# nubot-nudt/MDGAT-matcher

Hardware: AMD Instinct MI355X
Metric: keypoint-pairs/sec (higher is better)
Workload: dtype f32 (products as 3 split-f16 MFMAs, fp32 accumulate)

## Files before the change

mdgat_matcher_amd/csrc/attention_stream.hip:

```cpp
#include "common.hpp"
#include <utility>

namespace {

typedef float f32x2 __attribute__((ext_vector_type(2)));
typedef f16x8 __attribute__((may_alias)) f16x8_a;
typedef f32x4 __attribute__((may_alias)) f32x4_a;

constexpr int BLK_BYTES = 4096 + 128;
constexpr int CHUNK_BYTES = 4 * BLK_BYTES;
constexpr int NSLOT = 4;
constexpr int OROW = 36;

struct StreamArgs {
    const _Float16* q16;
    const _Float16* k16;
    const _Float16* vt16;
    float* msg;
    int N, M, Npad, PP, cross, QT;
};

template <typename F, int... U>
__device__ __forceinline__ void for_each_unit(F&& f, std::integer_sequence<int, U...>) { (f(U), ...); }
template <int N, typename F>
__device__ __forceinline__ void for_units(F&& f) { for_each_unit(f, std::make_integer_sequence<int, N>{}); }

#define SLOT_END() __builtin_amdgcn_sched_barrier(0)

template <bool FAST, bool QK_ONLY = false>
__global__ __launch_bounds__(256, 2) void attention_stream_kernel(StreamArgs a) {
    extern __shared__ __attribute__((aligned(16))) char smem[];
    const int tid = threadIdx.x, lane = tid & 63;
    const int wave = __builtin_amdgcn_readfirstlane(tid >> 6);
    const int l31 = lane & 31, hi = lane >> 5;
    const int i0 = blockIdx.x;
    const int grp = (i0 / (8 * a.QT)) * 8 + (i0 & 7), qt = (i0 >> 3) % a.QT;
    const int head = grp & 3, side = (grp >> 2) & 1, b = grp >> 3;
    const int P = a.N + a.M;
    const int nq = side ? a.M : a.N, q_off = side ? a.N : 0;
    const int src = a.cross ? 1 - side : side;
    const int nk = src ? a.M : a.N, k_off = src ? a.N : 0;
    const int q0 = qt * 128;
    if (q0 >= nq) return;
    const int NCH = nk >> 6;
    const unsigned lds0 = (unsigned)(size_t)(__attribute__((address_space(3))) char*)smem;

    const int rl8 = lane >> 3, swz = (lane & 7) ^ rl8;
    const char* dbase;
    unsigned voff, pstride, cstride;
    if (wave < 2) {
        dbase = reinterpret_cast<const char*>(a.k16 + (((size_t)b * P + k_off + wave * 32) * 4 + head) * 64);
        voff = rl8 * 512 + swz * 16; pstride = 8 * 512; cstride = 64 * 512;
    } else {
        dbase = reinterpret_cast<const char*>(a.vt16 + (((size_t)b * 4 + head) * 2 + (wave - 2)) * 32 * a.PP + (src ? a.Npad : 0));
        voff = rl8 * a.PP * 2 + swz * 16; pstride = 8 * a.PP * 2; cstride = 128;
    }
    auto dma_chunk = [&](int ch) __attribute__((always_inline)) {
        if (FAST && wave == 3) return;
        if (QK_ONLY && wave >= 2) return;
        const char* s0 = dbase + (size_t)ch * cstride;
        const unsigned d0 = lds0 + (unsigned)(ch & (NSLOT - 1)) * CHUNK_BYTES + (unsigned)wave * BLK_BYTES;
#pragma unroll
        for (int p = 0; p < 4; ++p)
            asm volatile("s_mov_b32 m0, %0\n\ts_nop 0\n\tglobal_load_lds_dwordx4 %1, %2"
                         :: "s"(d0 + p * 1024 + ((p >> 1) & 1) * 128), "v"(voff), "s"(s0 + (size_t)p * pstride) : "memory");
    };

    const int krow = (l31 & ~12) | ((l31 & 4) << 1) | ((l31 & 8) >> 1);
    unsigned kofs[4], vofs[4];
#pragma unroll
    for (int i = 0; i < 4; ++i) {
        const int c = 2 * i + hi;
        kofs[i] = (krow >> 3) * 1024 + ((krow >> 4) & 1) * 128 + ((krow & 7) * 8 + (c ^ (krow & 7))) * 16;
        vofs[i] = (l31 >> 3) * 1024 + ((l31 >> 4) & 1) * 128 + ((l31 & 7) * 8 + (c ^ (l31 & 7))) * 16;
    }
    f16x8 kf[4];
    f16x8 vh[2], vl[2];
    auto kread = [&](int ch, int jb) __attribute__((always_inline)) {
        const char* base = smem + (ch & (NSLOT - 1)) * CHUNK_BYTES + jb * BLK_BYTES;
#pragma unroll
        for (int i = 0; i < (FAST ? 2 : 4); ++i) kf[i] = *reinterpret_cast<const f16x8_a*>(base + kofs[i]);
    };
    auto vread = [&](int ch, int i) __attribute__((always_inline)) {
        if (QK_ONLY) return;
        const char* base = smem + (ch & (NSLOT - 1)) * CHUNK_BYTES + 2 * BLK_BYTES;
        vh[i & 1] = *reinterpret_cast<const f16x8_a*>(base + vofs[i]);
        if (!FAST) vl[i & 1] = *reinterpret_cast<const f16x8_a*>(base + BLK_BYTES + vofs[i]);
    };

    const int qw = q0 + wave * 32;
    f16x8 qh[2], ql[2];
    {
        const int qrow = min(qw + l31, nq - 1);
        const _Float16* p = a.q16 + (((size_t)b * P + q_off + qrow) * 4 + head) * 64 + 8 * hi;
        qh[0] = *reinterpret_cast<const f16x8*>(p);
        qh[1] = *reinterpret_cast<const f16x8*>(p + 16);
        ql[0] = *reinterpret_cast<const f16x8*>(p + 32);
        ql[1] = *reinterpret_cast<const f16x8*>(p + 48);
    }
    dma_chunk(0);
    if (NCH > 1) dma_chunk(1);
    if (NCH > 2) dma_chunk(2);
    if (NCH > 2) asm volatile("s_waitcnt vmcnt(8)" ::: "memory");
    else if (NCH > 1) asm volatile("s_waitcnt vmcnt(4)" ::: "memory");
    else asm volatile("s_waitcnt vmcnt(0)" ::: "memory");
    __syncthreads();

    const float NEG_INF = -__builtin_inff();
    const f32x16 zero16 = {0.f, 0.f, 0.f, 0.f, 0.f, 0.f, 0.f, 0.f, 0.f, 0.f, 0.f, 0.f, 0.f, 0.f, 0.f, 0.f};
    f32x16 Sc[2];
    f32x16 A, X;
    f32x16 Om = zero16;
    f32x2 l2 = {0.f, 0.f};
    float mxa = NEG_INF, mxb = NEG_INF;

    auto qk = [&](int k) __attribute__((always_inline)) {
        if (k == 0) A = __builtin_amdgcn_mfma_f32_32x32x16_f16(kf[0], qh[0], zero16, 0, 0, 0);
        else if (FAST) { if (k == 2) A = __builtin_amdgcn_mfma_f32_32x32x16_f16(kf[1], qh[1], A, 0, 0, 0); }
        else if (k == 1) X = __builtin_amdgcn_mfma_f32_32x32x16_f16(kf[0], ql[0], zero16, 0, 0, 0);
        else if (k == 2) A = __builtin_amdgcn_mfma_f32_32x32x16_f16(kf[1], qh[1], A, 0, 0, 0);
        else if (k == 3) X = __builtin_amdgcn_mfma_f32_32x32x16_f16(kf[1], ql[1], X, 0, 0, 0);
        else if (k == 4) X = __builtin_amdgcn_mfma_f32_32x32x16_f16(kf[2], qh[0], X, 0, 0, 0);
        else X = __builtin_amdgcn_mfma_f32_32x32x16_f16(kf[3], qh[1], X, 0, 0, 0);
    };
    auto comb = [&](int jb, int u) __attribute__((always_inline)) {
        if (u < 2) {
#pragma unroll
            for (int r = 8 * u; r < 8 * u + 8; r += 2) {
                if (FAST) { Sc[jb][r] = A[r]; Sc[jb][r + 1] = A[r + 1]; continue; }
                const f32x2 v = f32x2{X[r], X[r + 1]} + f32x2{A[r], A[r + 1]};
                Sc[jb][r] = v[0]; Sc[jb][r + 1] = v[1];
            }
        } else {
            const int r0 = 8 * (u - 2);
            mxa = fmaxf(mxa, fmaxf(Sc[jb][r0], Sc[jb][r0 + 1]));
            mxb = fmaxf(mxb, fmaxf(Sc[jb][r0 + 2], Sc[jb][r0 + 3]));
            mxa = fmaxf(mxa, fmaxf(Sc[jb][r0 + 4], Sc[jb][r0 + 5]));
            mxb = fmaxf(mxb, fmaxf(Sc[jb][r0 + 6], Sc[jb][r0 + 7]));
        }
    };

    for_units<2>([&](int jb) __attribute__((always_inline)) {
        kread(0, jb);
        for_units<6>([&](int k) __attribute__((always_inline)) { qk(k); });
        for_units<4>([&](int u) __attribute__((always_inline)) { comb(jb, u); });
    });
    float m_run;
    {
        float mc = fmaxf(mxa, mxb);
        m_run = fmaxf(mc, __shfl_xor(mc, 32, 64));
    }

    float pv[8];
    f16x8 php[2], plp[2];
#pragma unroll
    for (int j = 0; j < 8; ++j) { php[1][j] = (_Float16)0.f; plp[1][j] = (_Float16)0.f; vh[1][j] = (_Float16)0.f; vl[1][j] = (_Float16)0.f; }
    float m11 = 0.f;
    typedef unsigned u32x4 __attribute__((ext_vector_type(4)));
    auto vs = [&](int i, int u) __attribute__((always_inline)) {
        if (QK_ONLY) return;
        const int jb = i >> 1, r0 = 8 * (i & 1), pb = i & 1;
        if (u == 0) {
#pragma unroll
            for (int j = 0; j < 8; j += 2) {
                const f32x2 d = f32x2{Sc[jb][r0 + j], Sc[jb][r0 + j + 1]} - f32x2{m11, m11};
                pv[j] = d[0]; pv[j + 1] = d[1];
            }
        } else if (u == 1 || u == 2) {
#pragma unroll
            for (int j = 4 * (u - 1); j < 4 * u; ++j) pv[j] = __builtin_amdgcn_exp2f(pv[j]);
        } else if (u == 3) {
#pragma unroll
            for (int j = 0; j < 8; j += 2) l2 += f32x2{pv[j], pv[j + 1]};
        } else if (u == 4) {
#pragma unroll
            for (int j = 0; j < 8; ++j) php[pb][j] = (_Float16)pv[j];
        } else if (FAST) {
        } else if (u == 5 || u == 6) {
            const u32x4 hp = __builtin_bit_cast(u32x4, php[pb]);
#pragma unroll
            for (int j = 2 * (u - 5); j < 2 * (u - 4); ++j) {
                asm("v_fma_mix_f32 %0, %1, 1.0, -%2 op_sel:[0,0,0] op_sel_hi:[0,0,1]" : "=v"(pv[2 * j]) : "v"(pv[2 * j]), "v"(hp[j]));
                asm("v_fma_mix_f32 %0, %1, 1.0, -%2 op_sel:[0,0,1] op_sel_hi:[0,0,1]" : "=v"(pv[2 * j + 1]) : "v"(pv[2 * j + 1]), "v"(hp[j]));
            }
        } else {
#pragma unroll
            for (int j = 0; j < 8; ++j) plp[pb][j] = (_Float16)pv[j];
        }
    };
    auto pvm = [&](int i, int k) __attribute__((always_inline)) {
        if (QK_ONLY) return;
        const int pb = i & 1;
        if (k == 0) Om = __builtin_amdgcn_mfma_f32_32x32x16_f16(vh[pb], php[pb], Om, 0, 0, 0);
        else if (FAST) {}
        else if (k == 1) Om = __builtin_amdgcn_mfma_f32_32x32x16_f16(vl[pb], php[pb], Om, 0, 0, 0);
        else Om = __builtin_amdgcn_mfma_f32_32x32x16_f16(vh[pb], plp[pb], Om, 0, 0, 0);
    };

    auto max_halves = [&](float v) __attribute__((always_inline)) {
        float a_ = v, b_ = v;
        asm volatile("s_nop 1\n\tv_permlane32_swap_b32 %0, %1\n\ts_nop 1" : "+v"(a_), "+v"(b_));
        return fmaxf(a_, b_);
    };
    float sc = 1.0f;
    auto chunk_body = [&](int c, auto next_tag) __attribute__((always_inline)) {
        constexpr bool NEXT = decltype(next_tag)::value;
        if (c + 2 < NCH) asm volatile("s_waitcnt vmcnt(4)" ::: "memory");
        else asm volatile("s_waitcnt vmcnt(0)" ::: "memory");
        __syncthreads();
        if (c + 3 < NCH) dma_chunk(c + 3);
        if (NEXT) kread(c + 1, 0);
        m11 = m_run - 11.0f;
        mxa = NEG_INF; mxb = NEG_INF;
        l2 *= sc;
        SLOT_END();
        pvm(3, 0); vs(0, 0); SLOT_END();
        pvm(3, 1); vs(0, 1); SLOT_END();
        pvm(3, 2); vread(c, 0); SLOT_END();
        for_units<6>([&](int k) __attribute__((always_inline)) {
            if (NEXT) qk(k);
            vs(0, 2 + k);
            if (k == 3) vread(c, 1);
            SLOT_END();
        });
        if (!__all(sc == 1.0f)) {
#pragma unroll
            for (int r = 0; r < 16; ++r) Om[r] *= sc;
        }
        SLOT_END();
        if (NEXT) kread(c + 1, 1);
        for_units<8>([&](int u) __attribute__((always_inline)) {
            if (u < 3) pvm(0, u);
            vs(1, u);
            if (NEXT && u >= 3 && u < 7) comb(0, u - 3);
            if (u == 5) vread(c, 2);
            SLOT_END();
        });
        for_units<8>([&](int u) __attribute__((always_inline)) {
            if (NEXT && u < 6) qk(u);
            SLOT_END();
            if (u >= 1 && u < 4) pvm(1, u - 1);
            vs(2, u);
            if (u == 6) vread(c, 3);
            SLOT_END();
        });
        for_units<8>([&](int u) __attribute__((always_inline)) {
            if (u < 3) pvm(2, u);
            vs(3, u);
            if (NEXT && u >= 3 && u < 7) comb(1, u - 3);
            SLOT_END();
        });
        if (NEXT) {
            float mc = fmaxf(mxa, mxb);
            mc = max_halves(mc);
            const float m_new = mc > m_run + 4.0f ? mc : m_run;
            sc = __builtin_amdgcn_exp2f(m_run - m_new);
            m_run = m_new;
        }
    };
    for (int c = 0; c + 1 < NCH; ++c) chunk_body(c, std::true_type{});
    chunk_body(NCH - 1, std::false_type{});
    for_units<3>([&](int k) __attribute__((always_inline)) { pvm(3, k); });
    if (QK_ONLY) {
        if (hi == 0 && qw + l31 < nq) a.msg[((size_t)b * P + q_off + qw + l31) * 128 + head * 32] = m_run;
        return;
    }

    float l = l2[0] + l2[1];
    l += __shfl_xor(l, 32, 64);
    const float inv_l = 1.0f / l;
    float* T = reinterpret_cast<float*>(smem + ((NCH + 2 - (wave >> 1)) & (NSLOT - 1)) * CHUNK_BYTES) + (wave & 1) * 32 * OROW;
#pragma unroll
    for (int g4 = 0; g4 < 4; ++g4) {
        f32x4 o;
#pragma unroll
        for (int j = 0; j < 4; ++j) o[j] = Om[4 * g4 + j] * inv_l;
        *reinterpret_cast<f32x4_a*>(T + l31 * OROW + 8 * g4 + 4 * hi) = o;
    }
    float* out = a.msg + ((size_t)b * P + q_off) * 128 + head * 32;
#pragma unroll
    for (int it = 0; it < 4; ++it) {
        const int row = it * 8 + (lane >> 3), cc = lane & 7;
        const f32x4 v = *reinterpret_cast<const f32x4_a*>(T + row * OROW + cc * 4);
        const int q = qw + row;
        if (q < nq) *reinterpret_cast<f32x4*>(out + (size_t)q * 128 + cc * 4) = v;
    }
}


template <int NQ>
__global__ __launch_bounds__(256, 2) void qk_phase_probe_kernel(StreamArgs a) {
    extern __shared__ __attribute__((aligned(16))) char smem[];
    const int tid = threadIdx.x, lane = tid & 63;
    const int wave = __builtin_amdgcn_readfirstlane(tid >> 6);
    const int l31 = lane & 31, hi = lane >> 5;
    const int i0 = blockIdx.x;
    const int grp = (i0 / (8 * a.QT)) * 8 + (i0 & 7), qt = (i0 >> 3) % a.QT;
    const int head = grp & 3, side = (grp >> 2) & 1, b = grp >> 3;
    const int P = a.N + a.M;
    const int nq = side ? a.M : a.N, q_off = side ? a.N : 0;
    const int src = a.cross ? 1 - side : side;
    const int nk = src ? a.M : a.N, k_off = src ? a.N : 0;
    const int q0 = qt * 128 * NQ;
    if (q0 >= nq) return;
    const int NCH = nk >> 6;
    const unsigned lds0 = (unsigned)(size_t)(__attribute__((address_space(3))) char*)smem;
    const int rl8 = lane >> 3, swz = (lane & 7) ^ rl8;
    const char* dbase = reinterpret_cast<const char*>(a.k16 + (((size_t)b * P + k_off + (wave & 1) * 32) * 4 + head) * 64);
    const unsigned voff = rl8 * 512 + swz * 16;
    auto dma_chunk = [&](int ch) __attribute__((always_inline)) {
        if (wave >= 2) return;
        const char* s0 = dbase + (size_t)ch * (64 * 512);
        const unsigned d0 = lds0 + (unsigned)(ch & (NSLOT - 1)) * CHUNK_BYTES + (unsigned)wave * BLK_BYTES;
#pragma unroll
        for (int p = 0; p < 4; ++p)
            asm volatile("s_mov_b32 m0, %0\n\ts_nop 0\n\tglobal_load_lds_dwordx4 %1, %2"
                         :: "s"(d0 + p * 1024 + ((p >> 1) & 1) * 128), "v"(voff), "s"(s0 + (size_t)p * (8 * 512)) : "memory");
    };
    const int krow = (l31 & ~12) | ((l31 & 4) << 1) | ((l31 & 8) >> 1);
    unsigned kofs[4];
#pragma unroll
    for (int i = 0; i < 4; ++i) {
        const int c = 2 * i + hi;
        kofs[i] = (krow >> 3) * 1024 + ((krow >> 4) & 1) * 128 + ((krow & 7) * 8 + (c ^ (krow & 7))) * 16;
    }
    const int qw = q0 + wave * 32 * NQ;
    f16x8 qh[NQ][2], ql[NQ][2];
#pragma unroll
    for (int s_ = 0; s_ < NQ; ++s_) {
        const int qrow = min(qw + 32 * s_ + l31, nq - 1);
        const _Float16* p = a.q16 + (((size_t)b * P + q_off + qrow) * 4 + head) * 64 + 8 * hi;
        qh[s_][0] = *reinterpret_cast<const f16x8*>(p);
        qh[s_][1] = *reinterpret_cast<const f16x8*>(p + 16);
        ql[s_][0] = *reinterpret_cast<const f16x8*>(p + 32);
        ql[s_][1] = *reinterpret_cast<const f16x8*>(p + 48);
    }
    dma_chunk(0);
    if (NCH > 1) dma_chunk(1);
    if (NCH > 2) dma_chunk(2);
    const f32x16 zero16 = {0.f, 0.f, 0.f, 0.f, 0.f, 0.f, 0.f, 0.f, 0.f, 0.f, 0.f, 0.f, 0.f, 0.f, 0.f, 0.f};
    float mx[NQ];
#pragma unroll
    for (int s_ = 0; s_ < NQ; ++s_) mx[s_] = -__builtin_inff();
    for (int c = 0; c < NCH; ++c) {
        if (wave < 2) {
            if (c + 2 < NCH) asm volatile("s_waitcnt vmcnt(8)" ::: "memory");
            else if (c + 1 < NCH) asm volatile("s_waitcnt vmcnt(4)" ::: "memory");
            else asm volatile("s_waitcnt vmcnt(0)" ::: "memory");
        } else if (c == 0) asm volatile("s_waitcnt vmcnt(0)" ::: "memory");
        __syncthreads();
        if (c + 3 < NCH) dma_chunk(c + 3);
#pragma unroll
        for (int jb = 0; jb < 2; ++jb) {
            const char* base = smem + (c & (NSLOT - 1)) * CHUNK_BYTES + jb * BLK_BYTES;
            f16x8 kf[4];
#pragma unroll
            for (int i = 0; i < 4; ++i) kf[i] = *reinterpret_cast<const f16x8_a*>(base + kofs[i]);
            f32x16 A[NQ], X[NQ];
#pragma unroll
            for (int s_ = 0; s_ < NQ; ++s_) A[s_] = __builtin_amdgcn_mfma_f32_32x32x16_f16(kf[0], qh[s_][0], zero16, 0, 0, 0);
#pragma unroll
            for (int s_ = 0; s_ < NQ; ++s_) X[s_] = __builtin_amdgcn_mfma_f32_32x32x16_f16(kf[0], ql[s_][0], zero16, 0, 0, 0);
#pragma unroll
            for (int s_ = 0; s_ < NQ; ++s_) A[s_] = __builtin_amdgcn_mfma_f32_32x32x16_f16(kf[1], qh[s_][1], A[s_], 0, 0, 0);
#pragma unroll
            for (int s_ = 0; s_ < NQ; ++s_) X[s_] = __builtin_amdgcn_mfma_f32_32x32x16_f16(kf[1], ql[s_][1], X[s_], 0, 0, 0);
#pragma unroll
            for (int s_ = 0; s_ < NQ; ++s_) X[s_] = __builtin_amdgcn_mfma_f32_32x32x16_f16(kf[2], qh[s_][0], X[s_], 0, 0, 0);
#pragma unroll
            for (int s_ = 0; s_ < NQ; ++s_) X[s_] = __builtin_amdgcn_mfma_f32_32x32x16_f16(kf[3], qh[s_][1], X[s_], 0, 0, 0);
#pragma unroll
            for (int s_ = 0; s_ < NQ; ++s_)
#pragma unroll
                for (int r = 0; r < 16; r += 2) {
                    const f32x2 v = f32x2{X[s_][r], X[s_][r + 1]} + f32x2{A[s_][r], A[s_][r + 1]};
                    mx[s_] = fmaxf(mx[s_], fmaxf(v[0], v[1]));
                }
        }
    }
#pragma unroll
    for (int s_ = 0; s_ < NQ; ++s_) {
        const float m = fmaxf(mx[s_], __shfl_xor(mx[s_], 32, 64));
        const int q = qw + 32 * s_ + l31;
        if (hi == 0 && q < nq) a.msg[((size_t)b * P + q_off + q) * 128 + head * 32] = m;
    }
}

}

bool attention_stream_supported(int N, int M) { return N % 64 == 0 && M % 64 == 0; }

int launch_attention_stream(int B, int N, int M, int cross, const Qkv16& qkv, float* msg, hipStream_t s, int mode) {
    StreamArgs a{qkv.q16, qkv.k16, qkv.vt16, msg, N, M, qkv.Npad, qkv.PP, cross, attention_stream_qtiles(N, M)};
    const size_t lds = (size_t)NSLOT * CHUNK_BYTES;
    static std::atomic<unsigned long long> optin[2];
    const void* kern = mode == 1 ? reinterpret_cast<const void*>(attention_stream_kernel<true>) : reinterpret_cast<const void*>(attention_stream_kernel<false>);
    if (int rc = mdgat_lds_optin(kern, lds, optin[mode == 1], "attention LDS attribute")) return rc;
    if (mode == 1) hipLaunchKernelGGL(attention_stream_kernel<true>, dim3(B * 8 * a.QT), dim3(256), lds, s, a);
    else hipLaunchKernelGGL(attention_stream_kernel<false>, dim3(B * 8 * a.QT), dim3(256), lds, s, a);
    attention_count_launch(mode == 1 ? ATTN_STREAM_FAST : ATTN_STREAM);
    return mdgat_check_hip(hipGetLastError(), "attention launch");
}

int launch_attention_qk_probe(int B, int N, int M, int cross, const Qkv16& qkv, float* msg, hipStream_t s) {
    if (!attention_stream_supported(N, M)) { mdgat_set_error("qk probe: key counts must be multiples of 64"); return MDGAT_ERR_UNSUPPORTED; }
    const int nq_max = N > M ? N : M;
    StreamArgs a{qkv.q16, qkv.k16, qkv.vt16, msg, N, M, qkv.Npad, qkv.PP, cross, (nq_max + 127) / 128};
    const size_t lds = (size_t)NSLOT * CHUNK_BYTES;
    static std::atomic<unsigned long long> optin;
    if (int rc = mdgat_lds_optin(reinterpret_cast<const void*>(attention_stream_kernel<false, true>), lds, optin, "qk probe LDS attribute")) return rc;
    hipLaunchKernelGGL((attention_stream_kernel<false, true>), dim3(B * 8 * a.QT), dim3(256), lds, s, a);
    return mdgat_check_hip(hipGetLastError(), "qk probe launch");
}

int launch_qk_phase_probe(int B, int N, int M, int cross, int nq_sets, const Qkv16& qkv, float* msg, hipStream_t s) {
    if (!attention_stream_supported(N, M)) { mdgat_set_error("qk probe: key counts must be multiples of 64"); return MDGAT_ERR_UNSUPPORTED; }
    if (nq_sets != 1 && nq_sets != 2) { mdgat_set_error("qk probe: nq_sets must be 1 or 2"); return MDGAT_ERR_BAD_ARG; }
    const int nq_max = N > M ? N : M;
    const int per_wg = 128 * nq_sets;
    StreamArgs a{qkv.q16, qkv.k16, qkv.vt16, msg, N, M, qkv.Npad, qkv.PP, cross, (nq_max + per_wg - 1) / per_wg};
    const size_t lds = (size_t)NSLOT * CHUNK_BYTES;
    static std::atomic<unsigned long long> optin[2];
    const void* kern = nq_sets == 2 ? reinterpret_cast<const void*>(qk_phase_probe_kernel<2>) : reinterpret_cast<const void*>(qk_phase_probe_kernel<1>);
    if (int rc = mdgat_lds_optin(kern, lds, optin[nq_sets - 1], "qk phase probe LDS attribute")) return rc;
    if (nq_sets == 2) hipLaunchKernelGGL(qk_phase_probe_kernel<2>, dim3(B * 8 * a.QT), dim3(256), lds, s, a);
    else hipLaunchKernelGGL(qk_phase_probe_kernel<1>, dim3(B * 8 * a.QT), dim3(256), lds, s, a);
    return mdgat_check_hip(hipGetLastError(), "qk phase probe launch");
}
```

Measured before the change: 21340.

## Fold max-shift into QK accumulator seed and chain split-f16 MFMAs into one accumulator

QK split-f16 products now accumulate in a single MFMA chain rather than two partial accumulators that are added afterwards. The chain is seeded with -(m_run-11), so scores come out already shifted and the per-element subtract before exp2 goes away. Score tiles rotate through three register buffers and the chunk loop is unrolled by three with phase tags, which rebalances the slot schedule. Rescaling now happens only when a block max exceeds a fixed threshold, and the shift is applied to pending tiles. This changes numerical rounding order, raises register pressure from the extra tile and unroll, and the threshold rescale may behave differently from the old online-max rule.

```diff
diff --git a/mdgat_matcher_amd/csrc/attention_stream.hip b/mdgat_matcher_amd/csrc/attention_stream.hip
--- a/mdgat_matcher_amd/csrc/attention_stream.hip
+++ b/mdgat_matcher_amd/csrc/attention_stream.hip
@@ -108,70 +108,75 @@
 
     const float NEG_INF = -__builtin_inff();
     const f32x16 zero16 = {0.f, 0.f, 0.f, 0.f, 0.f, 0.f, 0.f, 0.f, 0.f, 0.f, 0.f, 0.f, 0.f, 0.f, 0.f, 0.f};
-    f32x16 Sc[2];
-    f32x16 A, X;
+    f32x16 S[3];
+    f32x16 Sd = zero16;
     f32x16 Om = zero16;
     f32x2 l2 = {0.f, 0.f};
     float mxa = NEG_INF, mxb = NEG_INF;
-
-    auto qk = [&](int k) __attribute__((always_inline)) {
-        if (k == 0) A = __builtin_amdgcn_mfma_f32_32x32x16_f16(kf[0], qh[0], zero16, 0, 0, 0);
-        else if (FAST) { if (k == 2) A = __builtin_amdgcn_mfma_f32_32x32x16_f16(kf[1], qh[1], A, 0, 0, 0); }
-        else if (k == 1) X = __builtin_amdgcn_mfma_f32_32x32x16_f16(kf[0], ql[0], zero16, 0, 0, 0);
-        else if (k == 2) A = __builtin_amdgcn_mfma_f32_32x32x16_f16(kf[1], qh[1], A, 0, 0, 0);
-        else if (k == 3) X = __builtin_amdgcn_mfma_f32_32x32x16_f16(kf[1], ql[1], X, 0, 0, 0);
-        else if (k == 4) X = __builtin_amdgcn_mfma_f32_32x32x16_f16(kf[2], qh[0], X, 0, 0, 0);
-        else X = __builtin_amdgcn_mfma_f32_32x32x16_f16(kf[3], qh[1], X, 0, 0, 0);
-    };
-    auto comb = [&](int jb, int u) __attribute__((always_inline)) {
-        if (u < 2) {
-#pragma unroll
-            for (int r = 8 * u; r < 8 * u + 8; r += 2) {
-                if (FAST) { Sc[jb][r] = A[r]; Sc[jb][r + 1] = A[r + 1]; continue; }
-                const f32x2 v = f32x2{X[r], X[r + 1]} + f32x2{A[r], A[r + 1]};
-                Sc[jb][r] = v[0]; Sc[jb][r + 1] = v[1];
-            }
-        } else {
-            const int r0 = 8 * (u - 2);
-            mxa = fmaxf(mxa, fmaxf(Sc[jb][r0], Sc[jb][r0 + 1]));
-            mxb = fmaxf(mxb, fmaxf(Sc[jb][r0 + 2], Sc[jb][r0 + 3]));
-            mxa = fmaxf(mxa, fmaxf(Sc[jb][r0 + 4], Sc[jb][r0 + 5]));
-            mxb = fmaxf(mxb, fmaxf(Sc[jb][r0 + 6], Sc[jb][r0 + 7]));
+    using T0 = std::integral_constant<int, 0>;
+    using T1 = std::integral_constant<int, 1>;
+    using T2 = std::integral_constant<int, 2>;
+
+    auto qk = [&](auto dst, auto seeded_tag, int k) __attribute__((always_inline)) {
+        constexpr int D = decltype(dst)::value;
+        constexpr bool HI_FIRST = decltype(seeded_tag)::value && !QK_ONLY;
+        if (FAST) {
+            if (k == 0) S[D] = __builtin_amdgcn_mfma_f32_32x32x16_f16(kf[0], qh[0], Sd, 0, 0, 0);
+            else if (k == 1) S[D] = __builtin_amdgcn_mfma_f32_32x32x16_f16(kf[1], qh[1], S[D], 0, 0, 0);
+            return;
         }
-    };
-
-    for_units<2>([&](int jb) __attribute__((always_inline)) {
-        kread(0, jb);
-        for_units<6>([&](int k) __attribute__((always_inline)) { qk(k); });
-        for_units<4>([&](int u) __attribute__((always_inline)) { comb(jb, u); });
-    });
+        const int p = HI_FIRST ? (k == 0 ? 5 : k == 1 ? 4 : k - 2) : k;
+        const f32x16 acc = k == 0 ? Sd : S[D];
+        if (p == 0) S[D] = __builtin_amdgcn_mfma_f32_32x32x16_f16(kf[0], ql[0], acc, 0, 0, 0);
+        else if (p == 1) S[D] = __builtin_amdgcn_mfma_f32_32x32x16_f16(kf[1], ql[1], acc, 0, 0, 0);
+        else if (p == 2) S[D] = __builtin_amdgcn_mfma_f32_32x32x16_f16(kf[2], qh[0], acc, 0, 0, 0);
+        else if (p == 3) S[D] = __builtin_amdgcn_mfma_f32_32x32x16_f16(kf[3], qh[1], acc, 0, 0, 0);
+        else if (p == 4) S[D] = __builtin_amdgcn_mfma_f32_32x32x16_f16(kf[0], qh[0], acc, 0, 0, 0);
+        else S[D] = __builtin_amdgcn_mfma_f32_32x32x16_f16(kf[1], qh[1], acc, 0, 0, 0);
+    };
+    auto bmax = [&](auto blk, int u) __attribute__((always_inline)) {
+        constexpr int D = decltype(blk)::value;
+        const int r0 = 8 * u;
+        mxa = fmaxf(fmaxf(mxa, S[D][r0]), S[D][r0 + 1]);
+        mxb = fmaxf(fmaxf(mxb, S[D][r0 + 2]), S[D][r0 + 3]);
+        mxa = fmaxf(fmaxf(mxa, S[D][r0 + 4]), S[D][r0 + 5]);
+        mxb = fmaxf(fmaxf(mxb, S[D][r0 + 6]), S[D][r0 + 7]);
+    };
+
+    kread(0, 0);
+    for_units<6>([&](int k) __attribute__((always_inline)) { qk(T0{}, std::false_type{}, k); });
+    for_units<2>([&](int u) __attribute__((always_inline)) { bmax(T0{}, u); });
+    kread(0, 1);
+    for_units<6>([&](int k) __attribute__((always_inline)) { qk(T1{}, std::false_type{}, k); });
+    for_units<2>([&](int u) __attribute__((always_inline)) { bmax(T1{}, u); });
     float m_run;
     {
         float mc = fmaxf(mxa, mxb);
         m_run = fmaxf(mc, __shfl_xor(mc, 32, 64));
     }
+    if (!QK_ONLY) {
+        const float m11 = m_run - 11.0f;
+#pragma unroll
+        for (int r = 0; r < 16; ++r) { S[0][r] -= m11; S[1][r] -= m11; Sd[r] = -m11; }
+        asm volatile("" : "+v"(Sd));
+    }
 
     float pv[8];
     f16x8 php[2], plp[2];
 #pragma unroll
     for (int j = 0; j < 8; ++j) { php[1][j] = (_Float16)0.f; plp[1][j] = (_Float16)0.f; vh[1][j] = (_Float16)0.f; vl[1][j] = (_Float16)0.f; }
-    float m11 = 0.f;
     typedef unsigned u32x4 __attribute__((ext_vector_type(4)));
-    auto vs = [&](int i, int u) __attribute__((always_inline)) {
+    auto vs = [&](auto blk, int i, int u) __attribute__((always_inline)) {
         if (QK_ONLY) return;
-        const int jb = i >> 1, r0 = 8 * (i & 1), pb = i & 1;
-        if (u == 0) {
-#pragma unroll
-            for (int j = 0; j < 8; j += 2) {
-                const f32x2 d = f32x2{Sc[jb][r0 + j], Sc[jb][r0 + j + 1]} - f32x2{m11, m11};
-                pv[j] = d[0]; pv[j + 1] = d[1];
-            }
-        } else if (u == 1 || u == 2) {
-#pragma unroll
-            for (int j = 4 * (u - 1); j < 4 * u; ++j) pv[j] = __builtin_amdgcn_exp2f(pv[j]);
+        constexpr int D = decltype(blk)::value;
+        const int r0 = 8 * (i & 1), pb = i & 1;
+        if (u == 1 || u == 2) {
+#pragma unroll
+            for (int j = 4 * (u - 1); j < 4 * u; ++j) pv[j] = __builtin_amdgcn_exp2f(S[D][r0 + j]);
         } else if (u == 3) {
 #pragma unroll
             for (int j = 0; j < 8; j += 2) l2 += f32x2{pv[j], pv[j + 1]};
+            asm volatile("" : "+v"(l2));
         } else if (u == 4) {
 #pragma unroll
             for (int j = 0; j < 8; ++j) php[pb][j] = (_Float16)pv[j];
@@ -203,63 +208,85 @@
         return fmaxf(a_, b_);
     };
     float sc = 1.0f;
-    auto chunk_body = [&](int c, auto next_tag) __attribute__((always_inline)) {
+    auto chunk_body = [&](int c, auto next_tag, auto phase_tag) __attribute__((always_inline)) {
         constexpr bool NEXT = decltype(next_tag)::value;
+        constexpr int I0 = (3 - decltype(phase_tag)::value) % 3;
+        using B0 = std::integral_constant<int, I0>;
+        using B1 = std::integral_constant<int, (I0 + 1) % 3>;
+        using BP = std::integral_constant<int, (I0 + 2) % 3>;
         if (c + 2 < NCH) asm volatile("s_waitcnt vmcnt(4)" ::: "memory");
         else asm volatile("s_waitcnt vmcnt(0)" ::: "memory");
         __syncthreads();
         if (c + 3 < NCH) dma_chunk(c + 3);
         if (NEXT) kread(c + 1, 0);
-        m11 = m_run - 11.0f;
         mxa = NEG_INF; mxb = NEG_INF;
         l2 *= sc;
         SLOT_END();
-        pvm(3, 0); vs(0, 0); SLOT_END();
-        pvm(3, 1); vs(0, 1); SLOT_END();
-        pvm(3, 2); vread(c, 0); SLOT_END();
+        pvm(3, 0); vs(B0{}, 0, 1); SLOT_END();
+        pvm(3, 1); vs(B0{}, 0, 2); SLOT_END();
+        pvm(3, 2); vread(c, 0); vs(B0{}, 0, 3); SLOT_END();
         for_units<6>([&](int k) __attribute__((always_inline)) {
-            if (NEXT) qk(k);
-            vs(0, 2 + k);
+            if (NEXT) qk(BP{}, std::true_type{}, k);
+            if (k < 4) vs(B0{}, 0, 4 + k);
             if (k == 3) vread(c, 1);
+            if (k == 4 && !QK_ONLY && !__all(sc == 1.0f)) {
+#pragma unroll
+                for (int r = 0; r < 16; ++r) Om[r] *= sc;
+            }
+            if (k == 5) vs(B0{}, 1, 1);
             SLOT_END();
         });
-        if (!__all(sc == 1.0f)) {
-#pragma unroll
-            for (int r = 0; r < 16; ++r) Om[r] *= sc;
-        }
-        SLOT_END();
         if (NEXT) kread(c + 1, 1);
-        for_units<8>([&](int u) __attribute__((always_inline)) {
-            if (u < 3) pvm(0, u);
-            vs(1, u);
-            if (NEXT && u >= 3 && u < 7) comb(0, u - 3);
-            if (u == 5) vread(c, 2);
-            SLOT_END();
-        });
-        for_units<8>([&](int u) __attribute__((always_inline)) {
-            if (NEXT && u < 6) qk(u);
-            SLOT_END();
-            if (u >= 1 && u < 4) pvm(1, u - 1);
-            vs(2, u);
-            if (u == 6) vread(c, 3);
-            SLOT_END();
-        });
-        for_units<8>([&](int u) __attribute__((always_inline)) {
-            if (u < 3) pvm(2, u);
-            vs(3, u);
-            if (NEXT && u >= 3 && u < 7) comb(1, u - 3);
-            SLOT_END();
-        });
+        pvm(0, 0); vs(B0{}, 1, 2); SLOT_END();
+        pvm(0, 1); vs(B0{}, 1, 3); SLOT_END();
+        pvm(0, 2); vs(B0{}, 1, 4); if (NEXT) bmax(BP{}, 0); SLOT_END();
+        if (NEXT) qk(B0{}, std::true_type{}, 0); vs(B0{}, 1, 5); if (NEXT) bmax(BP{}, 1); vread(c, 2); SLOT_END();
+        if (NEXT) qk(B0{}, std::true_type{}, 1); vs(B0{}, 1, 6); SLOT_END();
+        if (NEXT) qk(B0{}, std::true_type{}, 2); vs(B0{}, 1, 7); SLOT_END();
+        pvm(1, 0); vs(B1{}, 2, 1); SLOT_END();
+        if (NEXT) qk(B0{}, std::true_type{}, 3); vs(B1{}, 2, 2); SLOT_END();
+        pvm(1, 1); vs(B1{}, 2, 3); SLOT_END();
+        if (NEXT) qk(B0{}, std::true_type{}, 4); vs(B1{}, 2, 4); SLOT_END();
+        pvm(1, 2); vs(B1{}, 2, 5); vread(c, 3); SLOT_END();
+        if (NEXT) qk(B0{}, std::true_type{}, 5); vs(B1{}, 2, 6); SLOT_END();
+        vs(B1{}, 2, 7); SLOT_END();
+        pvm(2, 0); vs(B1{}, 3, 1); SLOT_END();
+        vs(B1{}, 3, 2); SLOT_END();
+        pvm(2, 1); vs(B1{}, 3, 3); SLOT_END();
+        vs(B1{}, 3, 4); if (NEXT) bmax(B0{}, 0); SLOT_END();
+        pvm(2, 2); vs(B1{}, 3, 5); if (NEXT) bmax(B0{}, 1); SLOT_END();
+        vs(B1{}, 3, 6); SLOT_END();
+        vs(B1{}, 3, 7); SLOT_END();
         if (NEXT) {
             float mc = fmaxf(mxa, mxb);
             mc = max_halves(mc);
-            const float m_new = mc > m_run + 4.0f ? mc : m_run;
-            sc = __builtin_amdgcn_exp2f(m_run - m_new);
-            m_run = m_new;
+            if (QK_ONLY) m_run = fmaxf(m_run, mc);
+            else {
+                sc = 1.0f;
+                if (__any(mc > 15.0f)) {
+                    float d = mc > 15.0f ? mc - 11.0f : 0.0f;
+                    asm volatile("" : "+v"(d));
+#pragma unroll
+                    for (int r = 0; r < 16; ++r) { S[BP::value][r] -= d; S[B0::value][r] -= d; Sd[r] -= d; }
+                    asm volatile("" : "+v"(Sd));
+                    sc = __builtin_amdgcn_exp2f(-d);
+                    m_run += d;
+                }
+            }
         }
     };
-    for (int c = 0; c + 1 < NCH; ++c) chunk_body(c, std::true_type{});
-    chunk_body(NCH - 1, std::false_type{});
+    {
+        using Y = std::true_type;
+        using N_ = std::false_type;
+        int c = 0;
+        for (; c + 3 < NCH; c += 3) { chunk_body(c, Y{}, T0{}); chunk_body(c + 1, Y{}, T1{}); chunk_body(c + 2, Y{}, T2{}); }
+        const int rem = NCH - c;
+        if (rem >= 2) chunk_body(c, Y{}, T0{});
+        if (rem == 3) chunk_body(c + 1, Y{}, T1{});
+        if (rem == 1) chunk_body(NCH - 1, N_{}, T0{});
+        else if (rem == 2) chunk_body(NCH - 1, N_{}, T1{});
+        else chunk_body(NCH - 1, N_{}, T2{});
+    }
     for_units<3>([&](int k) __attribute__((always_inline)) { pvm(3, k); });
     if (QK_ONLY) {
         if (hi == 0 && qw + l31 < nq) a.msg[((size_t)b * P + q_off + qw + l31) * 128 + head * 32] = m_run;
@@ -356,26 +383,23 @@
             f16x8 kf[4];
 #pragma unroll
             for (int i = 0; i < 4; ++i) kf[i] = *reinterpret_cast<const f16x8_a*>(base + kofs[i]);
-            f32x16 A[NQ], X[NQ];
-#pragma unroll
-            for (int s_ = 0; s_ < NQ; ++s_) A[s_] = __builtin_amdgcn_mfma_f32_32x32x16_f16(kf[0], qh[s_][0], zero16, 0, 0, 0);
-#pragma unroll
-            for (int s_ = 0; s_ < NQ; ++s_) X[s_] = __builtin_amdgcn_mfma_f32_32x32x16_f16(kf[0], ql[s_][0], zero16, 0, 0, 0);
-#pragma unroll
-            for (int s_ = 0; s_ < NQ; ++s_) A[s_] = __builtin_amdgcn_mfma_f32_32x32x16_f16(kf[1], qh[s_][1], A[s_], 0, 0, 0);
-#pragma unroll
-            for (int s_ = 0; s_ < NQ; ++s_) X[s_] = __builtin_amdgcn_mfma_f32_32x32x16_f16(kf[1], ql[s_][1], X[s_], 0, 0, 0);
-#pragma unroll
-            for (int s_ = 0; s_ < NQ; ++s_) X[s_] = __builtin_amdgcn_mfma_f32_32x32x16_f16(kf[2], qh[s_][0], X[s_], 0, 0, 0);
-#pragma unroll
-            for (int s_ = 0; s_ < NQ; ++s_) X[s_] = __builtin_amdgcn_mfma_f32_32x32x16_f16(kf[3], qh[s_][1], X[s_], 0, 0, 0);
+            f32x16 Sq[NQ];
+#pragma unroll
+            for (int s_ = 0; s_ < NQ; ++s_) Sq[s_] = __builtin_amdgcn_mfma_f32_32x32x16_f16(kf[0], ql[s_][0], zero16, 0, 0, 0);
+#pragma unroll
+            for (int s_ = 0; s_ < NQ; ++s_) Sq[s_] = __builtin_amdgcn_mfma_f32_32x32x16_f16(kf[1], ql[s_][1], Sq[s_], 0, 0, 0);
+#pragma unroll
+            for (int s_ = 0; s_ < NQ; ++s_) Sq[s_] = __builtin_amdgcn_mfma_f32_32x32x16_f16(kf[2], qh[s_][0], Sq[s_], 0, 0, 0);
+#pragma unroll
+            for (int s_ = 0; s_ < NQ; ++s_) Sq[s_] = __builtin_amdgcn_mfma_f32_32x32x16_f16(kf[3], qh[s_][1], Sq[s_], 0, 0, 0);
+#pragma unroll
+            for (int s_ = 0; s_ < NQ; ++s_) Sq[s_] = __builtin_amdgcn_mfma_f32_32x32x16_f16(kf[0], qh[s_][0], Sq[s_], 0, 0, 0);
+#pragma unroll
+            for (int s_ = 0; s_ < NQ; ++s_) Sq[s_] = __builtin_amdgcn_mfma_f32_32x32x16_f16(kf[1], qh[s_][1], Sq[s_], 0, 0, 0);
 #pragma unroll
             for (int s_ = 0; s_ < NQ; ++s_)
 #pragma unroll
-                for (int r = 0; r < 16; r += 2) {
-                    const f32x2 v = f32x2{X[s_][r], X[s_][r + 1]} + f32x2{A[s_][r], A[s_][r + 1]};
-                    mx[s_] = fmaxf(mx[s_], fmaxf(v[0], v[1]));
-                }
+                for (int r = 0; r < 16; r += 2) mx[s_] = fmaxf(fmaxf(mx[s_], Sq[s_][r]), Sq[s_][r + 1]);
         }
     }
 #pragma unroll
```

Result: no change. 21330 (-0.0%).
